# MougyTestspace/hclib

Measured on AMD Instinct MI355X. Metric: UTS nodes/sec (tasks/sec) at 1/2/4/8 MI355X vs host-CPU HClib; forasync HBM GB/s, higher is better.
Workload: dtype u32; 1 GPU; test/uts T3L (-t 0 -b 2000 -q 0.200014 -m 5 -r 7) searched whole on 1 GPU (no split); nodes=111345631, bit_exact=True, parallelism=shard1 (hash-partitioned frontier, RCCL all-reduce of counts)

## Files before the change

hclib_amd/__init__.py:

```python
from __future__ import annotations

import ctypes as C
import os
from typing import Optional, Tuple

PKG = os.path.dirname(os.path.abspath(__file__))
LIB_PATH = os.environ.get("HCLIB_AMD_LIB") or os.path.join(PKG, "lib", "libhclib_amd.so")

HCLIB_HIP_OK = 0
FORASYNC_MODE_FLAT = 0
FORASYNC_MODE_RECURSIVE = 1
BODY_TRIAD_F32 = 1
BODY_IOTA_CHECK = 2
BODY_VISIT_COUNT = 3


class HclibError(RuntimeError):
    pass


class LoopDomain(C.Structure):

    _fields_ = [("low", C.c_int), ("high", C.c_int), ("stride", C.c_int), ("tile", C.c_int)]

# ... 77 lines not shown


class StrassenResult(C.Structure):

    _fields_ = [("tasks", C.c_uint64), ("splits", C.c_uint64), ("base", C.c_uint64), ("tiles", C.c_uint64),
                ("pre_bands", C.c_uint64), ("combine_bands", C.c_uint64), ("finishes", C.c_uint64),
                ("check_ins", C.c_uint64), ("workspace_bytes", C.c_uint64),
                ("kernel_ms", C.c_double), ("gflops", C.c_double)]


class AtomicViewStruct(C.Structure):

    _fields_ = [("slots", C.c_void_p), ("nslots", C.c_uint32), ("stride", C.c_uint32),
                ("dtype", C.c_int), ("op", C.c_int)]


EXPORTS_HIP = [
    "hclib_hip_init", "hclib_hip_finalize", "hclib_hip_device_memory_live", "hclib_hip_last_error",
    "hclib_hip_num_cus",
    "hclib_hip_version", "hclib_hip_forasync", "hclib_hip_forasync_triad_f32",
    "hclib_hip_num_workers", "hclib_hip_uts_search", "hclib_hip_uts_num_children_host",
    "hclib_hip_uts_bucket_check", "hclib_hip_sha1_calibrate",
    "hclib_hip_fib", "hclib_hip_sw", "hclib_hip_last_sched_counters", "hclib_hip_last_narrow_counters",
    "hclib_hip_last_phase_counters",
    "hclib_hip_sw_band_begin", "hclib_hip_sw_band_rows", "hclib_hip_sw_band_end",
    "hclib_hip_atomic_create", "hclib_hip_atomic_destroy", "hclib_hip_atomic_view",
    "hclib_hip_atomic_gather", "hclib_hip_atomic_gather_async", "hclib_hip_atomic_reset",
    "hclib_hip_forasync_reduce", "hclib_hip_cholesky", "hclib_hip_sort_i64", "hclib_hip_sort_bounds",
    "hclib_hip_sparselu_genmat", "hclib_hip_sparselu_plan", "hclib_hip_sparselu", "hclib_hip_sparselu_bmod_rate",
    "hclib_hip_nqueens", "hclib_hip_nqueens_bounds",
    "hclib_hip_strassen", "hclib_hip_strassen_bounds", "hclib_hip_strassen_last_ticks",
    "hclib_atomic_create", "hclib_atomic_init", "hclib_atomic_update", "hclib_atomic_gather",
]

_lib = None


def lib():
    global _lib
    if _lib is None:
        try:
            import torch
        except ImportError:
            pass
        if not os.path.exists(LIB_PATH):
            raise HclibError(f"{LIB_PATH} is missing: run `python -m hclib_amd.build`")
        L = C.CDLL(LIB_PATH)
# ... 566 lines not shown
    _check(lib().hclib_hip_sha1_calibrate(chains, waves_per_cu, iters, C.byref(r), C.byref(ms)),
           "hclib_hip_sha1_calibrate")
    return r.value, ms.value


def last_phase_counters():
    out = (C.c_uint64 * 8)()
    lib().hclib_hip_last_phase_counters(out)
    return list(out)


def last_sched_counters():
    out = (C.c_uint64 * 16)()
    lib().hclib_hip_last_sched_counters(out)
    return list(out)


def last_narrow_counters():
    out = (C.c_uint64 * 4)()
    lib().hclib_hip_last_narrow_counters(out)
    return list(out)


TIMELINE_EVENTS = {1: "start", 2: "busy", 3: "idle", 4: "spill", 5: "term", 6: "end"}


def last_timeline():
    per = C.c_uint32()
    nw = lib().hclib_hip_last_timeline(None, 0, C.byref(per))
    if nw <= 0 or per.value == 0:
        return []
    import numpy as np
    buf = np.zeros(nw * per.value, dtype=np.uint64)
    lib().hclib_hip_last_timeline(buf.ctypes.data, buf.size, C.byref(per))
    buf = buf.reshape(nw, per.value)
    out = []
    for w in range(nw):
        row = buf[w][buf[w] != 0]
        out.append([(int(v >> 24), int((v >> 20) & 0xF), int(v & 0xFFFFF)) for v in row])
    return out
```

hclib_amd/csrc/hx_module.h:

```cpp
#pragma once

#include <hip/hip_runtime.h>
#include <stdint.h>

#include <string>
#include <vector>

#include "../../include/hclib_hip.h"
#include "../../include/hclib_hip/hx_sched.h"

namespace hx {

enum ArenaId {
    kArenaGlobals,
    kArenaWaveStats,
    kArenaWaveCtr,
    kArenaTimeline,
    kArenaDeques,
    kArenaSeed,
    kArenaDag,
    kArenaDagTrace,
    kArenaDyn,
    kArenaCholesky,
    kArenaSparselu,
    kArenaSort,
    kArenaStrassen,
    kArenaUtsTables,
    kArenaCount
};
struct Arena {
    void *mem = nullptr;
    size_t bytes = 0;
};

struct Module {
    bool inited = false;
    int device = -1;
    int num_cus = 0;
    std::string arch;
    hipStream_t stream = nullptr;
    hipEvent_t ev0 = nullptr, ev1 = nullptr;
    Arena arenas[kArenaCount];
    bool uts_tables_cached = false;
    SchedGlobals *globals = nullptr;
    unsigned long long last_counters[16] = {};
    unsigned long long last_narrow[4] = {};
    unsigned long long last_phase[8] = {};
    WaveStat *wave_stats = nullptr;
    uint32_t wave_stats_cap = 0;
    std::vector<WaveStat> last_waves;
    unsigned long long *wave_ctr = nullptr;
    uint32_t rec_workers = 0;
    GlobalView gview = {nullptr, nullptr, nullptr, 0, 0};
    unsigned long long *timeline = nullptr;
    uint32_t timeline_cap = 0;
    std::vector<unsigned long long> last_timeline;
};

Module &mod();
void set_error(const char *fmt, ...);
int ensure_device();
int hip_check(hipError_t e, const char *what);
int check_resident(const void *kern, int blocks, int threads, size_t lds, const char *what);
int upload_async(void *dst, const void *src, size_t bytes, hipStream_t stream);

int arena_reserve(ArenaId id, size_t bytes, const char *who, void **ptr);

class DevBuf {
  public:
// ... 31 lines not shown
```

hclib_amd/csrc/module.hip:

```cpp
#include <stdarg.h>
#include <stdio.h>
#include <stdlib.h>
#include <string.h>

#include "hx_module.h"

namespace hx {

static Module g_mod;
static thread_local char g_err[512] = "";

Module &mod() { return g_mod; }

void set_error(const char *fmt, ...) {
    va_list ap;
    va_start(ap, fmt);
    vsnprintf(g_err, sizeof(g_err), fmt, ap);
    va_end(ap);
}

static uint64_t g_live[2] = {0, 0};
static bool dev_acquire(void **p, size_t bytes) {
    if (hipMalloc(p, bytes) != hipSuccess) {
        (void)hipGetLastError();
// ... 211 lines not shown

int finish_sched(SchedGlobals *host_copy, const char *who) {
    Module &m = g_mod;
    HX_HIP(hipMemcpyAsync(host_copy, m.globals, sizeof(SchedGlobals), hipMemcpyDeviceToHost,
                          m.stream));
    const uint32_t nw_cap = m.wave_stats_cap;
    static std::vector<unsigned long long> rec;
    const uint32_t nrec = m.rec_workers;
    for (int i = 0; i < 8; ++i) m.last_phase[i] = 0;
    m.rec_workers = 0;
    if (nrec) {
        rec.resize((size_t)nrec * kWaveCtrWords);
        HX_HIP(hipMemcpyAsync(rec.data(), m.wave_ctr, rec.size() * 8, hipMemcpyDeviceToHost, m.stream));
    }
    HX_HIP(hipStreamSynchronize(m.stream));
    for (uint32_t w = 0; w < nrec; ++w) {
        const unsigned long long *r = &rec[(size_t)w * kWaveCtrWords];
        for (int i = 0; i < 16; ++i)
            if (i >= 8 || i < 4) host_copy->counters[i] += r[i];
        for (int i = 4; i < 8; ++i) host_copy->counters[i] += r[24 + i - 4];
        for (int i = 0; i < 4; ++i)
            if (r[16 + i] > host_copy->maxes[i]) host_copy->maxes[i] = r[16 + i];
        for (int i = 0; i < 3; ++i) host_copy->narrow[i] += r[20 + i];
        m.last_phase[0] += r[23];
        for (int i = 0; i < 4; ++i) m.last_phase[1 + i] += r[28 + i];
        m.last_phase[5] += r[24];
        m.last_phase[6] += r[27];
    }
    memcpy(m.last_counters, host_copy->counters, sizeof(m.last_counters));
    memcpy(m.last_narrow, host_copy->narrow, sizeof(m.last_narrow));
    uint64_t nw = host_copy->counters[kCtrWaves];
    if (nw > nw_cap) nw = nw_cap;
    m.last_waves.resize(nw);
    if (nw) HX_HIP(hipMemcpy(m.last_waves.data(), m.wave_stats, nw * sizeof(WaveStat), hipMemcpyDeviceToHost));
    if (host_copy->timeline) {
        m.last_timeline.resize((size_t)nw * m.timeline_cap);
        if (nw)
            HX_HIP(hipMemcpy(m.last_timeline.data(), m.timeline, (size_t)nw * m.timeline_cap * 8,
                             hipMemcpyDeviceToHost));
    } else {
        m.last_timeline.clear();
    }
    if (host_copy->err) {
        set_error("%s: device error %u (%s)", who, host_copy->err, err_name(host_copy->err));
        return HCLIB_HIP_EDEVICE;
    }
    return HCLIB_HIP_OK;
}

}

using namespace hx;

// ... 50 lines not shown
}

void hclib_hip_device_memory_live(uint64_t out[2]) {
    out[0] = g_live[0];
    out[1] = g_live[1];
}

int hclib_hip_num_cus(void) { return g_mod.inited ? g_mod.num_cus : 0; }

int hclib_hip_device(void) { return g_mod.inited ? g_mod.device : -1; }

void *hclib_hip_stream(void) { return g_mod.inited ? (void *)g_mod.stream : nullptr; }

void hclib_hip_last_sched_counters(uint64_t out[16]) {
    for (int i = 0; i < 16; ++i) out[i] = g_mod.last_counters[i];
}

extern "C" void hclib_hip_last_phase_counters(uint64_t out[8]) {
    for (int i = 0; i < 8; ++i) out[i] = g_mod.last_phase[i];
}

void hclib_hip_last_narrow_counters(uint64_t out[4]) {
    for (int i = 0; i < 4; ++i) out[i] = g_mod.last_narrow[i];
}

int hclib_hip_last_wave_stats(hclib_hip_wave_stats_t *out, int max) {
    static_assert(sizeof(hclib_hip_wave_stats_t) == sizeof(WaveStat), "layout");
    const int n = (int)g_mod.last_waves.size();
    for (int i = 0; out && i < n && i < max; ++i) memcpy(&out[i], &g_mod.last_waves[(size_t)i], sizeof(WaveStat));
    return n;
}

int hclib_hip_last_timeline(uint64_t *out, uint64_t max_words, uint32_t *events_per_worker) {
    Module &m = g_mod;
    if (events_per_worker) *events_per_worker = m.last_timeline.empty() ? 0u : m.timeline_cap;
    const uint64_t n = m.last_timeline.size();
    for (uint64_t i = 0; out && i < n && i < max_words; ++i) out[i] = m.last_timeline[i];
    return m.timeline_cap ? (int)(n / m.timeline_cap) : 0;
}

int hclib_hip_sched_begin(uint32_t entry_words, uint32_t chunk, int waves_per_cu,
                          hclib_hip_sched_launch_t *out) {
    if (!out || entry_words < 4 || entry_words > 64 || waves_per_cu < 1 || waves_per_cu > 8) {
        set_error("hclib_hip_sched_begin: invalid arguments");
        return HCLIB_HIP_EINVAL;
    }
// ... 183 lines not shown
```

hclib_amd/csrc/uts.hip:

```cpp
#include <math.h>
#include <string.h>

#include <type_traits>
#include <vector>

#include "hx_module.h"
#include "uts_sha1.h"

namespace hx {

#define HX_ROTL(x, n) (((x) << (n)) | ((x) >> (32 - (n))))
#define HX_RND(f, k, wi)                                \
    {                                                   \
        uint32_t t_ = HX_ROTL(a, 5) + (f) + e + (k) + (wi); \
        e = d;                                          \
        d = c;                                          \
        c = HX_ROTL(b, 30);                             \
        b = a;                                          \
        a = t_;                                         \
    }
#define HX_F1 (d ^ (b & (c ^ d)))
#define HX_F2 (b ^ c ^ d)
#define HX_F3 ((b & c) | (d & (b ^ c)))
#define HX_W(i) \
// ... 731 lines not shown
    }
    const bool seeded = seed_fits;
    if (seeded) spill_lo_default = uts_expected_nodes(*params) >= 3e7 ? 448 : 336;
    {
        const int ring_launch = bin ? 1024 : ring_used, lo = env_int("HCLIB_HIP_SPILL_LO", spill_lo_default);
        if (lo < 1 || lo > ring_launch) {
            set_error("hclib_hip_uts_search: HCLIB_HIP_SPILL_LO=%d does not fit the %d-item ring of this launch "
                      "(1..%d)", lo, ring_launch, ring_launch);
            return HCLIB_HIP_EINVAL;
        }
    }
    cfg.spill_lo = (uint32_t)env_int("HCLIB_HIP_SPILL_LO", spill_lo_default);
    cfg.spin_limit = (uint32_t)env_int("HCLIB_HIP_SPIN_LIMIT_MS", 20000);
    cfg.nwaves = (uint32_t)grid;
    cfg.stamps = (uint32_t)env_int("HCLIB_HIP_STAMPS", 0);
    const bool small_fixed = geo_fixed && uts_expected_nodes(*params) < 3e7;
    const bool large_fixed = geo_fixed && ring_used >= 512 && !small_fixed;
    cfg.hunger = (uint32_t)env_int("HCLIB_HIP_HUNGER", large_fixed ? 128 : bin ? 64 : 32);
    cfg.carry = (uint32_t)env_int("HCLIB_HIP_CARRY", 2);
    cfg.backoff = (uint32_t)env_int("HCLIB_HIP_BACKOFF", 16);
    cfg.defer = (uint32_t)env_int("HCLIB_HIP_DEFER", 1);
    cfg.dual = (uint32_t)env_int("HCLIB_HIP_UTS_DUAL", 1);
    cfg.spills = (uint32_t)env_int("HCLIB_HIP_SPILLS_PER_BATCH", 0);
    SeedCfg seed{0, 0, (uint32_t)UtsKind<kUtsBin, 0>::kWords, 0};
    if (seeded) {
        seed.target = (uint32_t)(grid * per_wave);
        seed.max_levels = (uint32_t)env_int("HCLIB_HIP_SEED_LEVELS", 20);
        seed.solo_cap = (uint32_t)env_int("HCLIB_HIP_SEED_SOLO", 128);
        if (nshards > 1) {
            double n_split = 1.0, n_next = 1.0;
            for (int d = 0; d <= split_depth && d < 64; ++d) {
                if (d < split_depth) n_split *= geo_bi(*params, d) > 0 ? geo_bi(*params, d) : 0.0;
                n_next *= geo_bi(*params, d) > 0 ? geo_bi(*params, d) : 0.0;
            }
            const double cap = 8.0 * seed.target + 65536.0;
            const bool fits = split_depth + 1 < kSeedMaxLevels && split_depth < (int)seed.max_levels &&
                              n_split <= 0.5 * cap && n_next / nshards <= (double)grid * (512 / 8);
            seed.min_levels = fits ? (uint32_t)split_depth : 0u;
        }
    } else if (bin_seed) {
        seed.target = 1;
        seed.max_levels = (uint32_t)split_depth;
        seed.min_levels = (uint32_t)split_depth;
    }
    HX_TRY(reset_sched(pool, 1, global, (uint32_t)grid, seed.target ? &seed : nullptr));
    HX_HIP(hipEventRecord(m.ev0, m.stream));
// ... 78 lines not shown
```

include/hclib_hip.h:

```cpp
#ifndef HCLIB_HIP_H_
#define HCLIB_HIP_H_

#include <stddef.h>
#include <stdint.h>

#ifdef __cplusplus
extern "C" {
#endif

#define HCLIB_HIP_OK 0
#define HCLIB_HIP_ENODEV (-1)
#define HCLIB_HIP_EINVAL (-2)
#define HCLIB_HIP_ENOMEM (-3)
#define HCLIB_HIP_EDEVICE (-4)
#define HCLIB_HIP_EHIP (-5)

int hclib_hip_init(int device);
void hclib_hip_finalize(void);
void hclib_hip_device_memory_live(uint64_t out[2]);
const char *hclib_hip_last_error(void);
int hclib_hip_num_cus(void);
int hclib_hip_device(void);
void *hclib_hip_stream(void);
const char *hclib_hip_version(void);
void hclib_hip_last_sched_counters(uint64_t out[16]);

typedef struct {
    uint64_t executed;
    uint64_t spawned;
    uint64_t batches;
    uint64_t chunks_pushed;
    uint64_t chunks_stolen;
    uint64_t items_stolen;
    uint64_t xcd;
    uint64_t reserved;
    uint64_t stolen_from[8];
} hclib_hip_wave_stats_t;
int hclib_hip_last_wave_stats(hclib_hip_wave_stats_t *out, int max);
void hclib_hip_last_narrow_counters(uint64_t out[4]);
void hclib_hip_last_phase_counters(uint64_t out[8]);
int hclib_hip_last_timeline(uint64_t *out, uint64_t max_words, uint32_t *events_per_worker);

#define HCLIB_HIP_ATOMIC_SCATTER_RET64 0
#define HCLIB_HIP_ATOMIC_HOT_WORD 1
#define HCLIB_HIP_ATOMIC_COALESCED32 2
int hclib_hip_atomic_calibrate(int mode, int iters, double *mops_per_s, double *kernel_ms);
int hclib_hip_sparselu_bmod_rate(int B, int wgs_per_cu, int reps, double *ms, double *gflops);
int hclib_hip_sha1_calibrate(int chains, int waves_per_cu, int iters, double *sha1_per_s, double *kernel_ms);

typedef struct {
    void *hdr;
    uint32_t *seq;
    uint32_t *cnt;
    uint32_t *data;
    uint32_t nq, cap, chunk;
    void *globals;
    void *stream;
    int grid;
    int num_cus;
} hclib_hip_sched_launch_t;

int hclib_hip_sched_begin(uint32_t entry_words, uint32_t chunk, int waves_per_cu,
// ... 272 lines not shown
```

include/hclib_hip/hx_sched.h:

```cpp
#pragma once

#include <type_traits>

#include "hx_common.h"

namespace hx {

constexpr int kWaveSize = 64;

struct alignas(256) QueueHdr {
    uint32_t head;
    uint32_t done;
    uint32_t pad0[30];
    uint32_t tail;
    uint32_t pad1[31];
};

struct WaveStat {
    unsigned long long executed, spawned, batches, chunks_pushed, chunks_stolen, items_stolen;
    unsigned long long xcd;
    unsigned long long reserved;
    unsigned long long stolen_from[8];
};
static_assert(sizeof(WaveStat) == 128, "WaveStat is 16 words");
// ... 29 lines not shown
    uint32_t pad1[63];
    uint32_t hints[8 * 64];
    uint32_t err;
    uint32_t pad2[63];
    unsigned long long counters[16];
    unsigned long long maxes[4];
    WaveStat *wave_stats;
    uint32_t wave_stats_cap;
    unsigned long long narrow[4];
    GlobalView gview;
    unsigned long long *timeline;
    uint32_t timeline_cap;
    unsigned long long *wave_ctr;
    uint32_t wave_ctr_cap;
    struct Seed {
        uint32_t *buf;
        uint32_t *ctl;
        uint32_t cap;
        uint32_t target;
        uint32_t max_levels;
        uint32_t min_levels;
        uint32_t solo_cap;
    } seed;
};
constexpr int kSeedMaxLevels = 24;
constexpr int kSeedGoLines = 64;
constexpr int kSeedCtlLines = 2 * kSeedMaxLevels + 2 + kSeedGoLines;
constexpr int kWaveCtrWords = 32;

#ifndef HX_TIMELINE
#define HX_TIMELINE 0
#endif
enum : uint32_t {
    kTlStart = 1,
    kTlBusy = 2,
    kTlIdle = 3,
    kTlSpill = 4,
    kTlTerm = 5,
    kTlEnd = 6,
    kTlProbe = 7,
    kTlSeed = 8,
};
struct Timeline {
    unsigned long long *p;
    uint32_t n, cap;
    __device__ __forceinline__ void init(SchedGlobals *g, uint32_t worker) {
#if HX_TIMELINE
        cap = g->timeline_cap;
        p = g->timeline ? g->timeline + (size_t)worker * cap : nullptr;
        n = 0;
#endif
// ... 30 lines not shown
struct PoolView {
    QueueHdr *hdr;
    uint32_t *seq;
    uint32_t *cnt;
    uint32_t *data;
    uint32_t nq;
    uint32_t cap;
    uint32_t chunk;
};

struct SchedConfig {
    uint32_t spill_hi;
    uint32_t spill_lo;
    uint32_t spin_limit;
    uint32_t nwaves;
    uint32_t stamps;
    uint32_t hunger;
    uint32_t backoff = 16;
    uint32_t carry = 2;
    uint32_t defer = 1;
    uint32_t dual = 1;
    uint32_t spills = 0;
    uint32_t hunger_init_full = 0;
};


constexpr uint32_t kResidualSplitMin = 2;

template <class K, class = void>
struct KindHasSeedProcess {
    static constexpr bool value = false;
};
template <class K>
struct KindHasSeedProcess<K, decltype((void)&K::seed_process)> {
    static constexpr bool value = true;
};
template <class K>
__device__ __forceinline__ int kind_seed_process(const typename K::Ctx &c, typename K::Acc &acc, const uint32_t *t,
                                                 uint32_t k, uint32_t *child, uint32_t *err, bool valid) {
    if constexpr (KindHasSeedProcess<K>::value) return K::seed_process(c, acc, t, k, child, err, valid);
    else return K::process(c, acc, t, k, child, err, valid);
}

template <class K, class = void>
struct KindPieces {
    static constexpr int value = 8;
// ... 12 lines not shown
struct KindHasDual<K, decltype((void)&K::process2)> {
    static constexpr bool value = K::kPure;
};
template <class K>
constexpr int group_max_of() { return KindPieces<K>::value + 2; }
template <class K, class = void>
struct KindFixedChildren {
    static constexpr bool value = false;
};
template <class K, class = void>
struct KindBulkCount {
    static constexpr bool value = false;
};
template <class K>
struct KindBulkCount<K, decltype((void)K::kBulkCount)> {
    static constexpr bool value = K::kBulkCount;
};
template <class K>
struct KindFixedChildren<K, decltype((void)K::kFixedChildren)> {
    static constexpr bool value = K::kFixedChildren;
};
constexpr uint32_t kMaxChildren = 1u << 24;

template <class Kind, int CAP>
struct WaveStack {
    static constexpr int TW = Kind::kTmplWords;
    static_assert(TW == 2 || TW == 6, "templates are 2 or 6 words");
    static_assert((CAP & (CAP - 1)) == 0, "CAP must be a power of two");
    uint2 d[CAP];
    uint4 t0[TW == 6 ? CAP : 1];
    uint2 t1[CAP];
    uint32_t mark[64];
    uint32_t stolen_from[8];
    unsigned long long cyc[6];
    static constexpr bool kCarryLds = CAP >= 1024;
    uint4 cscr[kCarryLds ? 128 : 1];
};

template <class WS>
__device__ __forceinline__ void lds_sum(WS &st, int i, unsigned long long v) {
    if (lane_id() == 0) __hip_atomic_fetch_add(&st.cyc[i], v, __ATOMIC_RELAXED, __HIP_MEMORY_SCOPE_WAVEFRONT);
}

template <class Kind, int CAP>
__device__ __forceinline__ void load_tmpl(const WaveStack<Kind, CAP> &st, uint32_t slot, uint32_t *t) {
    if constexpr (Kind::kTmplWords == 6) {
        const uint4 a = st.t0[slot];
        const uint2 b = st.t1[slot];
// ... 399 lines not shown
__device__ __forceinline__ uint32_t rcp16(uint32_t mu) {
    return mu <= 4 ? (mu <= 2 ? (mu == 1 ? 65536u : 32768u) : (mu == 3 ? 21846u : 16384u))
                   : (mu <= 6 ? (mu == 5 ? 13108u : 10923u) : (mu == 7 ? 9363u : 8192u));
}

template <int TW>
__device__ __forceinline__ void carry_permute(unsigned long long spawn, uint32_t mu, uint32_t nch,
                                              const uint32_t *child, uint32_t *ctmpl, uint32_t &ck,
                                              uint32_t rcp = 0) {
    const uint32_t lane = (uint32_t)lane_id();
    const uint32_t nsp = (uint32_t)__builtin_popcountll(spawn);
    const uint32_t rk = (uint32_t)__builtin_amdgcn_mbcnt_hi((uint32_t)(spawn >> 32),
                                                           __builtin_amdgcn_mbcnt_lo((uint32_t)spawn, 0u));
    const uint32_t dst = nch != 0 ? rk : nsp + (lane - rk);
    const int src_of_rank = __builtin_amdgcn_ds_permute((int)(dst * 4u), (int)lane);
    const uint32_t r = __umul24(lane, rcp ? rcp : rcp16(mu)) >> 16;
    const int src = __builtin_amdgcn_ds_bpermute((int)(r * 4u), src_of_rank);
#pragma unroll
    for (int i = 0; i < TW; ++i) ctmpl[i] = (uint32_t)__builtin_amdgcn_ds_bpermute(src * 4, (int)child[i]);
    ck = lane - __umul24(r, mu);
}

template <int TW>
__device__ __forceinline__ void carry_lds_slot(uint4 *scr, unsigned long long spawn, bool mine, const uint32_t *child,
                                               uint32_t *ctmpl, uint32_t r) {
    const uint32_t rk = (uint32_t)__builtin_amdgcn_mbcnt_hi((uint32_t)(spawn >> 32),
                                                           __builtin_amdgcn_mbcnt_lo((uint32_t)spawn, 0u));
    if (mine) {
        if constexpr (TW == 6) {
            scr[2 * rk] = make_uint4(child[0], child[1], child[2], child[3]);
            *(uint2 *)&scr[2 * rk + 1] = make_uint2(child[4], child[5]);
        } else {
            *(uint2 *)&scr[2 * rk] = make_uint2(child[0], child[1]);
        }
    }
    if constexpr (TW == 6) {
        const uint4 a = scr[2 * r];
        const uint2 b = *(const uint2 *)&scr[2 * r + 1];
        ctmpl[0] = a.x;
        ctmpl[1] = a.y;
        ctmpl[2] = a.z;
        ctmpl[3] = a.w;
        ctmpl[4] = b.x;
        ctmpl[5] = b.y;
    } else {
        const uint2 a = *(const uint2 *)&scr[2 * r];
        ctmpl[0] = a.x;
        ctmpl[1] = a.y;
    }
}

template <int TW>
__device__ __forceinline__ void carry_lds(uint4 *scr, unsigned long long spawn, uint32_t mu, const uint32_t *child,
                                          uint32_t *ctmpl, uint32_t &ck, uint32_t rcp = 0) {
    const uint32_t lane = (uint32_t)lane_id();
    const uint32_t r = __umul24(lane, rcp ? rcp : rcp16(mu)) >> 16;
    carry_lds_slot<TW>(scr, spawn, ((spawn >> lane) & 1ull) != 0, child, ctmpl, r);
    ck = lane - __umul24(r, mu);
}

template <class Kind, int CAP>
__device__ __forceinline__ void push_uniform(WaveStack<Kind, CAP> &st, uint32_t base, uint32_t excl,
                                             uint32_t tout, uint32_t mu, bool spawned,
                                             const uint32_t *child) {
    constexpr uint32_t M = CAP - 1;
    if (spawned) store_tmpl<Kind, CAP>(st, (base + excl) & M, child);
    const uint32_t rcp = rcp16(mu);
    for (uint32_t r0 = 0; r0 < tout; r0 += kWaveSize) {
        const uint32_t o = r0 + (uint32_t)lane_id();
        if (o < tout) {
            const uint32_t kk = o - ((o * rcp) >> 16) * mu;
            st.d[(base + o) & M] = make_uint2(kk, (kk + 1) | (kk << 24));
// ... 85 lines not shown
#endif
template <class A, class = void>
struct acc_has_mode : std::false_type {};
template <class A>
struct acc_has_mode<A, decltype((void)A::mode)> : std::true_type {};
template <class A>
__device__ __forceinline__ void acc_set_mode(A &a, uint32_t m) {
    if constexpr (acc_has_mode<A>::value) a.mode = m;
}
template <class A, class = void>
struct acc_has_totals : std::false_type {};
template <class A>
struct acc_has_totals<A, decltype((void)&A::totals)> : std::true_type {};

template <class A, class = void>
struct acc_has_wid : std::false_type {};
template <class A>
struct acc_has_wid<A, decltype((void)A::wid)> : std::true_type {};
template <class A>
__device__ __forceinline__ void acc_set_wid(A &a, uint32_t w) {
    if constexpr (acc_has_wid<A>::value) a.wid = w;
}

template <class Kind, int CAP>
__device__ __forceinline__ NarrowState<Kind::kTmplWords> narrow_loop_fixed(
    const typename Kind::Ctx &ctx_ref, typename Kind::Acc &acc_ref, uint32_t *err, WaveStack<Kind, CAP> &st,
    NarrowState<Kind::kTmplWords> ns, uint32_t mu, uint32_t r_fix, uint32_t ck_fix) {
    constexpr int TW = Kind::kTmplWords;
    const typename Kind::Ctx ctx = ctx_ref;
    typename Kind::Acc acc = acc_ref;
    acc_set_mode(acc, 1u);
    const uint32_t lane = (uint32_t)lane_id();
    constexpr bool kBulk = KindBulkCount<Kind>::value;
    uint32_t carry = lane0(ns.carry), batches = 0, s_exec = 0, s_nsp = 0, t2;
    const uint32_t k = ck_fix;
    uint32_t ch2[TW];
    bool sp;
    unsigned long long sp2;
    do {
        const bool h = lane < carry;
        if constexpr (kBulk) sp = Kind::process_bulk(ctx, acc, ns.ctmpl, k, ch2, err, h);
        else sp = Kind::process(ctx, acc, ns.ctmpl, k, ch2, err, h) > 0;
        ++batches;
        s_exec += carry;
        sp2 = __builtin_amdgcn_ballot_w64(sp);
        const uint32_t nsp = (uint32_t)__builtin_popcountll(sp2);
        s_nsp += nsp;
        t2 = mu * nsp;
        carry_lds_slot<TW>(st.cscr, sp2, sp, ch2, ns.ctmpl, r_fix);
        carry = t2;
    } while (t2 - 1u < (uint32_t)kWaveSize);
    ns.ck = ck_fix;
    if (t2 != 0) {
        const uint32_t rk2 = (uint32_t)__builtin_amdgcn_mbcnt_hi(
            (uint32_t)(sp2 >> 32), __builtin_amdgcn_mbcnt_lo((uint32_t)sp2, 0u));
        push_uniform<Kind, CAP>(st, ns.top, mu * rk2, t2, mu, sp, ch2);
        ns.top += t2;
        carry = 0;
    }
    if constexpr (kBulk) Kind::count_bulk(acc, s_exec, s_exec - s_nsp);
    if (lane == 0) {
        ns.n_exec += s_exec;
        ns.n_spawn += mu * s_nsp;
    }
    ns.carry = carry;
    ns.batches = batches;
    acc_set_mode(acc, 0u);
    acc_ref = acc;
    return ns;
}

template <class Kind, int CAP>
__device__ __forceinline__ NarrowState<Kind::kTmplWords> narrow_loop(
    const typename Kind::Ctx &ctx_ref, typename Kind::Acc &acc_ref, uint32_t *err, WaveStack<Kind, CAP> &st,
    NarrowState<Kind::kTmplWords> ns) {
    constexpr int TW = Kind::kTmplWords;
    constexpr int kPieces = pieces_of<Kind>();
    const typename Kind::Ctx ctx = ctx_ref;
    typename Kind::Acc acc = acc_ref;
    acc_set_mode(acc, 1u);
    const uint32_t lane = (uint32_t)lane_id();
    uint32_t carry = lane0(ns.carry), batches = 0;
    uint32_t mu_fix = 0, rcp_fix = 0;
    if constexpr (KindFixedChildren<Kind>::value) {
        mu_fix = lane0(Kind::fixed_children(ctx));
        if (mu_fix > (uint32_t)kPieces) mu_fix = 0;
        rcp_fix = mu_fix ? rcp16(mu_fix) : 0u;
    }
    const bool hoist = mu_fix != 0;
    const uint32_t r_fix = hoist ? __umul24(lane, rcp_fix) >> 16 : 0u;
    const uint32_t ck_fix = hoist ? lane - __umul24(r_fix, mu_fix) : 0u;
    if constexpr (KindFixedChildren<Kind>::value && Kind::kPure && Kind::kBoundedChildren &&
                  WaveStack<Kind, CAP>::kCarryLds) {
        if (hoist) return narrow_loop_fixed<Kind, CAP>(ctx_ref, acc_ref, err, st, ns, mu_fix, r_fix, ck_fix);
    }
    while (true) {
        const bool h = lane < carry;
        uint32_t ch2[TW];
        int c2 = 0;
        if constexpr (Kind::kPure) {
            c2 = Kind::process(ctx, acc, ns.ctmpl, ns.ck, ch2, err, h);
        } else {
            if (h) c2 = Kind::process(ctx, acc, ns.ctmpl, ns.ck, ch2, err, true);
        }
        ++batches;
        uint32_t u2 = c2 > 0 ? (uint32_t)c2 : 0u;
        if (!Kind::kBoundedChildren && u2 >= kMaxChildren) {
            dev_error(err, kErrBadTask);
            u2 = 0;
        }
        ns.n_exec += h ? 1u : 0u;
        ns.n_spawn += h ? u2 : 0u;
        const uint32_t n2 = u2 > (uint32_t)kPieces ? (uint32_t)kPieces : u2;
        const unsigned long long sp2 = __ballot(n2 != 0);
        if (!sp2) {
            carry = 0;
            break;
// ... 33 lines not shown
                                    ns.ck + 1, ns.tag);
            ns.tag += 16;
            ns.top += t2;
        }
        carry = 0;
        break;
    }
    ns.carry = carry;
    ns.batches = batches;
    acc_set_mode(acc, 0u);
    acc_ref = acc;
    return ns;
}

template <class Kind>
struct Inbox {
    uint32_t state;
    uint32_t n;
    uint32_t idle;
    uint32_t pad;
    uint32_t w[64 * Kind::kWords];
};

template <class Kind, int CAP>
__device__ bool inbox_put(const typename Kind::Ctx &ctx, Inbox<Kind> &ib, WaveStack<Kind, CAP> &st, uint32_t bot,
                          uint32_t n, SchedGlobals *g) {
    constexpr int W = Kind::kWords;
    const int lane = lane_id();
    const bool valid = (uint32_t)lane < n;
    const uint32_t p = bot + (valid ? (uint32_t)lane : 0u);
    const uint2 dd = st.d[p & (CAP - 1)];
    uint32_t ok = 0;
    if (lane == 0) ok = lds_cas(&ib.state, 0u, 2u) ? 1u : 0u;
    uint32_t w[W];
    load_tmpl<Kind, CAP>(st, (p - (dd.y >> 24)) & (CAP - 1), w);
    if (!lane0(ok)) return false;
    {
        w[W - 2] = dd.x;
        w[W - 1] = dd.y & (kMaxChildren - 1);
        kind_export<Kind>(ctx, w, valid, &g->err);
        kind_trace_item<Kind>(ctx, w, valid, 2u, true);
        if (valid) {
#pragma unroll
            for (int i = 0; i < W; ++i) ib.w[(uint32_t)lane * W + i] = w[i];
        }
    }
    asm volatile("" ::: "memory");
    if (lane == 0) {
        add_agent(&g->outstanding, 1u);
        lds_store(&ib.n, n);
        lds_store(&ib.idle, 0u);
        lds_store(&ib.state, 1u);
    }
    return true;
}

template <class Kind, int CAP>
__device__ uint32_t inbox_take(const typename Kind::Ctx &ctx, Inbox<Kind> &ib, WaveStack<Kind, CAP> &st) {
    constexpr int W = Kind::kWords;
    const int lane = lane_id();
    if (lane0(lds_load(&ib.state)) != 1u) return 0;
    const uint32_t n = lane0(lds_load(&ib.n));
    if ((uint32_t)lane < n) {
        uint32_t w[W];
#pragma unroll
        for (int i = 0; i < W; ++i) w[i] = ib.w[(uint32_t)lane * W + i];
        store_tmpl<Kind, CAP>(st, (uint32_t)lane, w);
        st.d[lane] = make_uint2(w[W - 2], w[W - 1]);
        kind_trace_item<Kind>(ctx, w, true, 3u, true);
    }
    if (lane == 0) lds_store(&ib.state, 0u);
    return n;
}

template <bool GLOBAL>
__device__ __forceinline__ void wave_goes_idle(SchedGlobals *g, const GlobalView &gv, const PoolView &pool) {
    if (lane_id() != 0) return;
// ... 241 lines not shown
    const uint32_t qpx = pool.nq / 8;
    const uint32_t xcc = xcc_id() & 7u;
    const uint32_t home = xcc * qpx + (gid / 8) % qpx;
    uint32_t rng = 0x9e3779b9u ^ (gid * 0x85ebca6bu + 1u);

    typename Kind::Acc acc;
    acc_set_wid(acc, gid);
    Timeline tl;
    tl.init(g, gid);
    tl.log(kTlStart, 0);
    ProbeStats pstat;
    uint32_t bot = 0, top = 0;
    bool active = false;
    uint32_t spins = 0;
    unsigned long long idle_since = 0;
    uint32_t nbatch = 0, npush = 0, nsteal = 0;
    unsigned long long cyc_form = 0, cyc_proc = 0, cyc_push = 0;
    unsigned long long ph_sum[6] = {0, 0, 0, 0, 0, 0}, ph_n = 0, ph_a = 0, ph_b = 0, ph_c = 0, ph_d = 0, ph_m = 0,
                       ph_p = 0;
    bool ph_single = false;
    uint32_t tag = 1;
    for (int i = lane; i < kWaveSize; i += kWaveSize) st.mark[i] = 0;
    if (lane < 8) st.stolen_from[lane] = 0;
    uint32_t n_exec = 0, n_spawn = 0;
    uint32_t items_stolen = 0;
    uint32_t n_narrow = 0, n_narrow_in = 0;
    uint32_t carry = 0, ck = 0;
    uint32_t ctmpl[TW];
    PendingChunk pend;
    pend.live = false;
    uint32_t occ = 0;
#pragma unroll
    for (int i = 0; i < TW; ++i) ctmpl[i] = 0;

    bool seeded = false;
    if constexpr (Kind::kPure && Kind::kTmplWords == 6 && Kind::kWords == 8 && CAP >= 128) {
        if (g->seed.buf) {
            seeded = true;
            top = seed_levels<Kind, CAP>(ctx, acc, g, st, gid, cfg.nwaves, cfg.spin_limit, n_exec, n_spawn, nbatch, tl);
            st.mark[lane] = 0;
            active = true;
            tl.log(kTlBusy, top);
            if (top == 0) {
                active = false;
                wave_goes_idle<GLOBAL>(g, gv, pool);
            }
// ... 365 lines not shown
            excl = (uint32_t)(P - nout);
        }
        {
            const uint32_t hungry0 = cfg.nwaves > outst ? cfg.nwaves - outst : 0;
            if (cfg.carry && uniform && tout > 0 && tout <= (uint32_t)kWaveSize &&
                !(hungry0 > 0 && (top - bot) + tout >= cfg.spill_lo)) {
                if constexpr (WaveStack<Kind, CAP>::kCarryLds) carry_lds<TW>(st.cscr, spawn, mu, child, ctmpl, ck);
                else carry_permute<TW>(spawn, mu, nch, child, ctmpl, ck);
                carry = tout;
                if (HX_STAMPS && cfg.stamps) cyc_push += __builtin_amdgcn_s_memtime() - ts0;
                if (HX_STAMPS && cfg.stamps) t_batch = __builtin_amdgcn_s_memtime();
                if (cfg.carry > 1 && top == bot && cfg.spill_lo > (uint32_t)kWaveSize && !(HX_STAMPS && cfg.stamps)) {
                    const unsigned long long tn0 = __builtin_amdgcn_s_memtime();
                    NarrowState<TW> ns;
#pragma unroll
                    for (int i = 0; i < TW; ++i) ns.ctmpl[i] = ctmpl[i];
                    ns.ck = ck;
                    ns.carry = carry;
                    ns.top = top;
                    ns.tag = tag;
                    ns.n_exec = n_exec;
                    ns.n_spawn = n_spawn;
                    ns.batches = 0;
                    ns = narrow_loop<Kind, CAP>(ctx, acc, &g->err, st, ns);
#pragma unroll
                    for (int i = 0; i < TW; ++i) ctmpl[i] = ns.ctmpl[i];
                    ck = ns.ck;
                    carry = lane0(ns.carry);
                    top = lane0(ns.top);
                    tag = lane0(ns.tag);
                    n_exec = ns.n_exec;
                    n_spawn = ns.n_spawn;
                    nbatch += lane0(ns.batches);
                    n_narrow += lane0(ns.batches);
                    lds_sum(st, 3, __builtin_amdgcn_s_memtime() - tn0);
                    ++n_narrow_in;
                }
                continue;
            }
        }
        if (HX_PHASES) ph_m = __builtin_amdgcn_s_memtime();
        if (!make_room(tout)) break;
        if (uniform) {
            push_uniform<Kind, CAP>(st, top, excl, tout, mu, nch != 0, child);
        } else {
            push_outputs<Kind, CAP>(st, top, excl, tout, nres, ucnt, nch, tmpl, child, k, kend, tag);
            tag += 16;
// ... 59 lines not shown
            const unsigned long long ph_e = __builtin_amdgcn_s_memtime();
            ph_sum[0] += ph_b - ph_a;
            ph_sum[1] += ph_c - ph_b;
            ph_sum[2] += ph_d - ph_c;
            ph_sum[3] += ph_e - ph_d;
            ph_sum[4] += ph_m - ph_d;
            ph_sum[5] += ph_p - ph_m;
            ++ph_n;
        }
    }
    publish_pending<Kind, CAP>(pool, g, pend);
    if constexpr (WPG > 1) {
        if (lane == 0) {
            lds_store(&ib[wave].idle, 0u);
            (void)lds_cas(&ib[wave].state, 0u, 3u);
        }
    }
    const unsigned long long t_end = __builtin_amdgcn_s_memtime();
    const unsigned long long rt_end = __builtin_amdgcn_s_memrealtime();
    lds_sum(st, busy_phase ? 0 : 1, t_end - t_mark);
    __builtin_amdgcn_s_waitcnt(0xC07F);
    const unsigned long long cyc_busy = st.cyc[0], cyc_idle = st.cyc[1], cyc_spill = st.cyc[2],
                             cyc_narrow = st.cyc[3], t_begin = st.cyc[4], rt_begin = st.cyc[5];
    if (active) {
        wave_goes_idle<GLOBAL>(g, gv, pool);
    }
    const bool rec = g->wave_ctr && gid < g->wave_ctr_cap;
    unsigned long long kc[8] = {0, 0, 0, 0, 0, 0, 0, 0}, km[4] = {0, 0, 0, 0};
    if constexpr (acc_has_totals<typename Kind::Acc>::value) {
        acc.totals(kc, km);
        if (!rec && lane == 0) {
            for (int i = 0; i < 8; ++i)
                if (kc[i]) add_agent(&g->counters[i], kc[i]);
            for (int i = 0; i < 4; ++i)
                if (km[i]) __hip_atomic_fetch_max(&g->maxes[i], km[i], __ATOMIC_RELAXED, HX_AGENT);
        }
    } else {
        acc.flush(g);
    }
    {
        const unsigned long long ex = wave_sum((unsigned long long)n_exec),
                                 sp = wave_sum((unsigned long long)n_spawn);
        if (g->wave_stats && gid < g->wave_stats_cap && lane < 16) {
            unsigned long long v = 0;
            switch (lane) {
            case 0: v = ex; break;
            case 1: v = sp; break;
            case 2: v = nbatch; break;
            case 3: v = npush; break;
            case 4: v = nsteal; break;
            case 5: v = items_stolen; break;
            case 6: v = xcc; break;
            case 7: v = 0; break;
            default: v = st.stolen_from[lane - 8]; break;
            }
            ((unsigned long long *)&g->wave_stats[gid])[lane] = v;
        }
    }
    const unsigned long long c_push = (HX_STAMPS && cfg.stamps) ? cyc_push - cyc_proc : 0,
                             c_form = (HX_STAMPS && cfg.stamps) ? cyc_form : 0,
                             c_proc = (HX_STAMPS && cfg.stamps) ? cyc_proc : 0;
    if (rec) {
        unsigned long long v = 0;
#pragma unroll
        for (int i = 0; i < 8; ++i)
            if (lane == i) v = kc[i];
#pragma unroll
        for (int i = 0; i < 4; ++i)
            if (lane == 16 + i) v = km[i];
        switch (lane) {
        case 8 + kCtrProcCycles - 8: v = c_proc; break;
        case 8 + kCtrBusyCycles - 8: v = cyc_busy; break;
        case 8 + kCtrIdleCycles - 8: v = cyc_idle; break;
        case 8 + kCtrSpillCycles - 8: v = cyc_spill; break;
        case 8 + kCtrWaves - 8: v = 1; break;
        case 8 + kCtrBatches - 8: v = nbatch; break;
        case 8 + kCtrPushed - 8: v = npush; break;
        case 8 + kCtrStolen - 8: v = nsteal; break;
        case 20: v = n_narrow_in ? (unsigned long long)n_narrow : 0; break;
        case 21: v = n_narrow_in ? cyc_narrow : 0; break;
        case 22: v = n_narrow_in; break;
        case 23: v = ph_n; break;
        case 28: v = ph_sum[0]; break;
        case 29: v = ph_sum[1]; break;
        case 30: v = ph_sum[2]; break;
        case 31: v = ph_sum[3]; break;
        case 24 + kCtrPushCycles - 4: v = HX_PHASES ? ph_sum[4] : c_push; break;
        case 24 + kCtrClockTicks - 4: v = t_end - t_begin; break;
        case 24 + kCtrRealTicks - 4: v = rt_end - rt_begin; break;
        case 24 + kCtrFormCycles - 4: v = HX_PHASES ? ph_sum[5] : c_form; break;
        default: break;
        }
        if (lane < kWaveCtrWords) g->wave_ctr[(size_t)gid * kWaveCtrWords + lane] = v;
    } else {
        if (lane == 0 && n_narrow_in) {
            add_agent(&g->narrow[0], (unsigned long long)n_narrow);
            add_agent(&g->narrow[1], cyc_narrow);
            add_agent(&g->narrow[2], (unsigned long long)n_narrow_in);
        }
        if (lane == 0) {
            add_agent(&g->counters[kCtrBusyCycles], cyc_busy);
            if (HX_STAMPS && cfg.stamps) {
                add_agent(&g->counters[kCtrFormCycles], c_form);
                add_agent(&g->counters[kCtrProcCycles], c_proc);
                add_agent(&g->counters[kCtrPushCycles], c_push);
            }
            add_agent(&g->counters[kCtrIdleCycles], cyc_idle);
            add_agent(&g->counters[kCtrSpillCycles], cyc_spill);
            add_agent(&g->counters[kCtrWaves], 1ull);
            add_agent(&g->counters[kCtrBatches], (unsigned long long)nbatch);
            add_agent(&g->counters[kCtrPushed], (unsigned long long)npush);
            add_agent(&g->counters[kCtrStolen], (unsigned long long)nsteal);
            add_agent(&g->counters[kCtrClockTicks], t_end - t_begin);
            add_agent(&g->counters[kCtrRealTicks], rt_end - rt_begin);
        }
    }
    tl.log(kTlEnd, 0);
// ... 11 lines not shown
```

Measured before the change: 4.123 billion nodes/s.

## Shed narrow-loop spawns into idle sibling inboxes on narrow exit

When the fixed-children narrow loop exits with spawned children, the wave now keeps only part of them (half, a quarter, or what fits one carry pass, chosen by HCLIB_HIP_NARROW_SHED) and hands the rest straight to idle sibling waves' LDS inboxes in the same workgroup. If all the remaining children go to inboxes, the wave keeps running the narrow loop on the kept ones instead of pushing to its ring. The aim is to cut ring push traffic and idle time in sibling waves by redistributing work inside the workgroup. It adds LDS state reads, CAS claims and outstanding-counter atomics at every narrow exit, plus new shed counters that widen the per-wave counter record to 40 words.

```diff
diff --git a/hclib_amd/__init__.py b/hclib_amd/__init__.py
--- a/hclib_amd/__init__.py
+++ b/hclib_amd/__init__.py
@@ -123,7 +123,7 @@
     "hclib_hip_num_workers", "hclib_hip_uts_search", "hclib_hip_uts_num_children_host",
     "hclib_hip_uts_bucket_check", "hclib_hip_sha1_calibrate",
     "hclib_hip_fib", "hclib_hip_sw", "hclib_hip_last_sched_counters", "hclib_hip_last_narrow_counters",
-    "hclib_hip_last_phase_counters",
+    "hclib_hip_last_phase_counters", "hclib_hip_last_shed_counters",
     "hclib_hip_sw_band_begin", "hclib_hip_sw_band_rows", "hclib_hip_sw_band_end",
     "hclib_hip_atomic_create", "hclib_hip_atomic_destroy", "hclib_hip_atomic_view",
     "hclib_hip_atomic_gather", "hclib_hip_atomic_gather_async", "hclib_hip_atomic_reset",
@@ -736,6 +736,12 @@
     return list(out)
 
 
+def last_shed_counters():
+    out = (C.c_uint64 * 8)()
+    lib().hclib_hip_last_shed_counters(out)
+    return dict(zip(("exits", "placed", "blocks", "items", "fallbacks"), out))
+
+
 TIMELINE_EVENTS = {1: "start", 2: "busy", 3: "idle", 4: "spill", 5: "term", 6: "end"}
 
 
diff --git a/hclib_amd/csrc/hx_module.h b/hclib_amd/csrc/hx_module.h
--- a/hclib_amd/csrc/hx_module.h
+++ b/hclib_amd/csrc/hx_module.h
@@ -45,6 +45,7 @@
     SchedGlobals *globals = nullptr;
     unsigned long long last_counters[16] = {};
     unsigned long long last_narrow[4] = {};
+    unsigned long long last_shed[8] = {};
     unsigned long long last_phase[8] = {};
     WaveStat *wave_stats = nullptr;
     uint32_t wave_stats_cap = 0;
diff --git a/hclib_amd/csrc/module.hip b/hclib_amd/csrc/module.hip
--- a/hclib_amd/csrc/module.hip
+++ b/hclib_amd/csrc/module.hip
@@ -257,6 +257,7 @@
         for (int i = 0; i < 4; ++i)
             if (r[16 + i] > host_copy->maxes[i]) host_copy->maxes[i] = r[16 + i];
         for (int i = 0; i < 3; ++i) host_copy->narrow[i] += r[20 + i];
+        for (int i = 0; i < kShedCounts; ++i) host_copy->shed[i] += r[32 + i];
         m.last_phase[0] += r[23];
         for (int i = 0; i < 4; ++i) m.last_phase[1 + i] += r[28 + i];
         m.last_phase[5] += r[24];
@@ -264,6 +265,7 @@
     }
     memcpy(m.last_counters, host_copy->counters, sizeof(m.last_counters));
     memcpy(m.last_narrow, host_copy->narrow, sizeof(m.last_narrow));
+    memcpy(m.last_shed, host_copy->shed, sizeof(m.last_shed));
     uint64_t nw = host_copy->counters[kCtrWaves];
     if (nw > nw_cap) nw = nw_cap;
     m.last_waves.resize(nw);
@@ -360,6 +362,10 @@
 
 void hclib_hip_last_narrow_counters(uint64_t out[4]) {
     for (int i = 0; i < 4; ++i) out[i] = g_mod.last_narrow[i];
+}
+
+void hclib_hip_last_shed_counters(uint64_t out[8]) {
+    for (int i = 0; i < 8; ++i) out[i] = g_mod.last_shed[i];
 }
 
 int hclib_hip_last_wave_stats(hclib_hip_wave_stats_t *out, int max) {
diff --git a/hclib_amd/csrc/uts.hip b/hclib_amd/csrc/uts.hip
--- a/hclib_amd/csrc/uts.hip
+++ b/hclib_amd/csrc/uts.hip
@@ -777,6 +777,15 @@
     cfg.defer = (uint32_t)env_int("HCLIB_HIP_DEFER", 1);
     cfg.dual = (uint32_t)env_int("HCLIB_HIP_UTS_DUAL", 1);
     cfg.spills = (uint32_t)env_int("HCLIB_HIP_SPILLS_PER_BATCH", 0);
+    {
+        const int rule = env_int("HCLIB_HIP_NARROW_SHED", 1), sibs = env_int("HCLIB_HIP_NARROW_SHED_SIBS", 3);
+        if (rule < 0 || rule > 3 || sibs < 0 || sibs > 3) {
+            set_error("hclib_hip_uts_search: HCLIB_HIP_NARROW_SHED=%d / HCLIB_HIP_NARROW_SHED_SIBS=%d: the keep rule is "
+                      "0 (off), 1, 2 or 3, the sibling inboxes per exit 0..3", rule, sibs);
+            return HCLIB_HIP_EINVAL;
+        }
+        cfg.narrow_shed = (uint32_t)rule | (uint32_t)sibs << 8;
+    }
     SeedCfg seed{0, 0, (uint32_t)UtsKind<kUtsBin, 0>::kWords, 0};
     if (seeded) {
         seed.target = (uint32_t)(grid * per_wave);
diff --git a/include/hclib_hip.h b/include/hclib_hip.h
--- a/include/hclib_hip.h
+++ b/include/hclib_hip.h
@@ -38,6 +38,7 @@
 } hclib_hip_wave_stats_t;
 int hclib_hip_last_wave_stats(hclib_hip_wave_stats_t *out, int max);
 void hclib_hip_last_narrow_counters(uint64_t out[4]);
+void hclib_hip_last_shed_counters(uint64_t out[8]);
 void hclib_hip_last_phase_counters(uint64_t out[8]);
 int hclib_hip_last_timeline(uint64_t *out, uint64_t max_words, uint32_t *events_per_worker);
 
diff --git a/include/hclib_hip/hx_sched.h b/include/hclib_hip/hx_sched.h
--- a/include/hclib_hip/hx_sched.h
+++ b/include/hclib_hip/hx_sched.h
@@ -75,11 +75,20 @@
         uint32_t min_levels;
         uint32_t solo_cap;
     } seed;
+    unsigned long long shed[8];
 };
 constexpr int kSeedMaxLevels = 24;
 constexpr int kSeedGoLines = 64;
 constexpr int kSeedCtlLines = 2 * kSeedMaxLevels + 2 + kSeedGoLines;
-constexpr int kWaveCtrWords = 32;
+constexpr int kWaveCtrWords = 40;
+enum : int {
+    kShedExits = 0,
+    kShedPlaced = 1,
+    kShedBlocks = 2,
+    kShedItems = 3,
+    kShedFallbacks = 4,
+    kShedCounts = 5,
+};
 
 #ifndef HX_TIMELINE
 #define HX_TIMELINE 0
@@ -156,6 +165,7 @@
     uint32_t dual = 1;
     uint32_t spills = 0;
     uint32_t hunger_init_full = 0;
+    uint32_t narrow_shed = 0;
 };
 
 
@@ -214,8 +224,19 @@
 };
 constexpr uint32_t kMaxChildren = 1u << 24;
 
+template <bool ON>
+struct ShedSlots {};
+template <>
+struct ShedSlots<true> {
+    unsigned long long shed_g;
+    uint32_t shed_ib;
+    uint32_t shed_wave;
+    uint32_t shed_cfg;
+    uint32_t shed_cnt[kShedCounts];
+};
+
 template <class Kind, int CAP>
-struct WaveStack {
+struct WaveStack : ShedSlots<(CAP >= 1024)> {
     static constexpr int TW = Kind::kTmplWords;
     static_assert(TW == 2 || TW == 6, "templates are 2 or 6 words");
     static_assert((CAP & (CAP - 1)) == 0, "CAP must be a power of two");
@@ -661,18 +682,7 @@
 }
 
 template <int TW>
-__device__ __forceinline__ void carry_lds_slot(uint4 *scr, unsigned long long spawn, bool mine, const uint32_t *child,
-                                               uint32_t *ctmpl, uint32_t r) {
-    const uint32_t rk = (uint32_t)__builtin_amdgcn_mbcnt_hi((uint32_t)(spawn >> 32),
-                                                           __builtin_amdgcn_mbcnt_lo((uint32_t)spawn, 0u));
-    if (mine) {
-        if constexpr (TW == 6) {
-            scr[2 * rk] = make_uint4(child[0], child[1], child[2], child[3]);
-            *(uint2 *)&scr[2 * rk + 1] = make_uint2(child[4], child[5]);
-        } else {
-            *(uint2 *)&scr[2 * rk] = make_uint2(child[0], child[1]);
-        }
-    }
+__device__ __forceinline__ void carry_lds_read(const uint4 *scr, uint32_t r, uint32_t *ctmpl) {
     if constexpr (TW == 6) {
         const uint4 a = scr[2 * r];
         const uint2 b = *(const uint2 *)&scr[2 * r + 1];
@@ -687,6 +697,21 @@
         ctmpl[0] = a.x;
         ctmpl[1] = a.y;
     }
+}
+template <int TW>
+__device__ __forceinline__ void carry_lds_slot(uint4 *scr, unsigned long long spawn, bool mine, const uint32_t *child,
+                                               uint32_t *ctmpl, uint32_t r) {
+    const uint32_t rk = (uint32_t)__builtin_amdgcn_mbcnt_hi((uint32_t)(spawn >> 32),
+                                                           __builtin_amdgcn_mbcnt_lo((uint32_t)spawn, 0u));
+    if (mine) {
+        if constexpr (TW == 6) {
+            scr[2 * rk] = make_uint4(child[0], child[1], child[2], child[3]);
+            *(uint2 *)&scr[2 * rk + 1] = make_uint2(child[4], child[5]);
+        } else {
+            *(uint2 *)&scr[2 * rk] = make_uint2(child[0], child[1]);
+        }
+    }
+    carry_lds_read<TW>(scr, r, ctmpl);
 }
 
 template <int TW>
@@ -818,7 +843,11 @@
     if constexpr (acc_has_wid<A>::value) a.wid = w;
 }
 
-template <class Kind, int CAP>
+template <class Kind, int CAP, int WPG>
+__device__ __forceinline__ uint32_t narrow_shed(const typename Kind::Ctx &ctx, WaveStack<Kind, CAP> &st, uint32_t mu,
+                                                uint32_t nsp, uint32_t r_fix, uint32_t ck_fix, uint32_t &to_ring);
+
+template <class Kind, int CAP, int WPG = 1>
 __device__ __forceinline__ NarrowState<Kind::kTmplWords> narrow_loop_fixed(
     const typename Kind::Ctx &ctx_ref, typename Kind::Acc &acc_ref, uint32_t *err, WaveStack<Kind, CAP> &st,
     NarrowState<Kind::kTmplWords> ns, uint32_t mu, uint32_t r_fix, uint32_t ck_fix) {
@@ -833,6 +862,7 @@
     uint32_t ch2[TW];
     bool sp;
     unsigned long long sp2;
+    while (true) {
     do {
         const bool h = lane < carry;
         if constexpr (kBulk) sp = Kind::process_bulk(ctx, acc, ns.ctmpl, k, ch2, err, h);
@@ -846,14 +876,19 @@
         carry_lds_slot<TW>(st.cscr, sp2, sp, ch2, ns.ctmpl, r_fix);
         carry = t2;
     } while (t2 - 1u < (uint32_t)kWaveSize);
+    if (t2 == 0) break;
+    const uint32_t nsp = (uint32_t)__builtin_popcountll(sp2);
+    uint32_t kept = 0, to_ring = 0;
+    if constexpr (WPG > 1) kept = narrow_shed<Kind, CAP, WPG>(ctx, st, mu, nsp, r_fix, ck_fix, to_ring);
+    carry = mu * kept;
+    if (kept != 0 && to_ring == nsp) continue;
+    const uint32_t rk2 = (uint32_t)__builtin_amdgcn_mbcnt_hi(
+        (uint32_t)(sp2 >> 32), __builtin_amdgcn_mbcnt_lo((uint32_t)sp2, 0u));
+    push_uniform<Kind, CAP>(st, ns.top, mu * (rk2 - to_ring), mu * (nsp - to_ring), mu, sp && rk2 >= to_ring, ch2);
+    ns.top += mu * (nsp - to_ring);
+    break;
+    }
     ns.ck = ck_fix;
-    if (t2 != 0) {
-        const uint32_t rk2 = (uint32_t)__builtin_amdgcn_mbcnt_hi(
-            (uint32_t)(sp2 >> 32), __builtin_amdgcn_mbcnt_lo((uint32_t)sp2, 0u));
-        push_uniform<Kind, CAP>(st, ns.top, mu * rk2, t2, mu, sp, ch2);
-        ns.top += t2;
-        carry = 0;
-    }
     if constexpr (kBulk) Kind::count_bulk(acc, s_exec, s_exec - s_nsp);
     if (lane == 0) {
         ns.n_exec += s_exec;
@@ -866,7 +901,7 @@
     return ns;
 }
 
-template <class Kind, int CAP>
+template <class Kind, int CAP, int WPG = 1>
 __device__ __forceinline__ NarrowState<Kind::kTmplWords> narrow_loop(
     const typename Kind::Ctx &ctx_ref, typename Kind::Acc &acc_ref, uint32_t *err, WaveStack<Kind, CAP> &st,
     NarrowState<Kind::kTmplWords> ns) {
@@ -888,7 +923,7 @@
     const uint32_t ck_fix = hoist ? lane - __umul24(r_fix, mu_fix) : 0u;
     if constexpr (KindFixedChildren<Kind>::value && Kind::kPure && Kind::kBoundedChildren &&
                   WaveStack<Kind, CAP>::kCarryLds) {
-        if (hoist) return narrow_loop_fixed<Kind, CAP>(ctx_ref, acc_ref, err, st, ns, mu_fix, r_fix, ck_fix);
+        if (hoist) return narrow_loop_fixed<Kind, CAP, WPG>(ctx_ref, acc_ref, err, st, ns, mu_fix, r_fix, ck_fix);
     }
     while (true) {
         const bool h = lane < carry;
@@ -968,6 +1003,33 @@
     uint32_t w[64 * Kind::kWords];
 };
 
+template <class Kind>
+__device__ __forceinline__ uint32_t inbox_claim(Inbox<Kind> &ib) {
+    uint32_t ok = 0;
+    if (lane_id() == 0) ok = lds_cas(&ib.state, 0u, 2u) ? 1u : 0u;
+    return ok;
+}
+
+template <class Kind>
+__device__ __forceinline__ void inbox_fill(const typename Kind::Ctx &ctx, Inbox<Kind> &ib, uint32_t *w, bool valid,
+                                           uint32_t n, SchedGlobals *g) {
+    constexpr int W = Kind::kWords;
+    kind_export<Kind>(ctx, w, valid, &g->err);
+    kind_trace_item<Kind>(ctx, w, valid, 2u, true);
+    if (valid) {
+        hx_lds_u32 *dst = (hx_lds_u32 *)&ib.w[(uint32_t)lane_id() * W];
+#pragma unroll
+        for (int i = 0; i < W; ++i) dst[i] = w[i];
+    }
+    asm volatile("" ::: "memory");
+    if (lane_id() == 0) {
+        add_agent(&g->outstanding, 1u);
+        lds_store(&ib.n, n);
+        lds_store(&ib.idle, 0u);
+        lds_store(&ib.state, 1u);
+    }
+}
+
 template <class Kind, int CAP>
 __device__ bool inbox_put(const typename Kind::Ctx &ctx, Inbox<Kind> &ib, WaveStack<Kind, CAP> &st, uint32_t bot,
                           uint32_t n, SchedGlobals *g) {
@@ -976,29 +1038,67 @@
     const bool valid = (uint32_t)lane < n;
     const uint32_t p = bot + (valid ? (uint32_t)lane : 0u);
     const uint2 dd = st.d[p & (CAP - 1)];
-    uint32_t ok = 0;
-    if (lane == 0) ok = lds_cas(&ib.state, 0u, 2u) ? 1u : 0u;
+    const uint32_t ok = inbox_claim<Kind>(ib);
     uint32_t w[W];
     load_tmpl<Kind, CAP>(st, (p - (dd.y >> 24)) & (CAP - 1), w);
     if (!lane0(ok)) return false;
-    {
-        w[W - 2] = dd.x;
-        w[W - 1] = dd.y & (kMaxChildren - 1);
-        kind_export<Kind>(ctx, w, valid, &g->err);
-        kind_trace_item<Kind>(ctx, w, valid, 2u, true);
-        if (valid) {
+    w[W - 2] = dd.x;
+    w[W - 1] = dd.y & (kMaxChildren - 1);
+    inbox_fill<Kind>(ctx, ib, w, valid, n, g);
+    return true;
+}
+
+template <class Kind, int CAP, int WPG>
+__device__ __forceinline__ uint32_t narrow_shed(const typename Kind::Ctx &ctx, WaveStack<Kind, CAP> &st, uint32_t mu,
+                                                uint32_t nsp, uint32_t r_fix, uint32_t ck_fix, uint32_t &to_ring) {
+    constexpr int TW = Kind::kTmplWords, W = Kind::kWords;
+    const uint32_t lane = (uint32_t)lane_id();
+    to_ring = 0;
+    const uint32_t cfg = lane0(lds_load(&st.shed_cfg));
+    const uint32_t rule = cfg & 0xffu, max_blocks = (cfg >> 8) & 0xffu;
+    if (rule == 0) return 0;
+    const uint32_t fit = (64u * rcp16(mu)) >> 16;
+    uint32_t keep = rule == 2 ? fit : (rule == 3 ? nsp / 4 : nsp / 2);
+    keep = keep > fit ? fit : (keep == 0 ? 1u : keep);
+    const uint32_t wave = lane0(lds_load(&st.shed_wave));
+    typedef __attribute__((address_space(3))) Inbox<Kind> lds_inbox;
+    Inbox<Kind> *ib = (Inbox<Kind> *)(lds_inbox *)(uintptr_t)lane0(lds_load(&st.shed_ib));
+    const unsigned long long gp = st.shed_g;
+    SchedGlobals *g = (SchedGlobals *)(((unsigned long long)lane0((uint32_t)(gp >> 32)) << 32) | lane0((uint32_t)gp));
+    uint32_t sid[WPG], sst[WPG];
 #pragma unroll
-            for (int i = 0; i < W; ++i) ib.w[(uint32_t)lane * W + i] = w[i];
-        }
-    }
-    asm volatile("" ::: "memory");
+    for (uint32_t a = 1; a < (uint32_t)WPG; ++a) {
+        sid[a] = lds_load(&ib[(wave + a) % (uint32_t)WPG].idle);
+        sst[a] = lds_load(&ib[(wave + a) % (uint32_t)WPG].state);
+    }
+    const uint32_t nshed = nsp - keep;
+    uint32_t placed = 0, blocks = 0;
+#pragma unroll
+    for (uint32_t a = 1; a < (uint32_t)WPG; ++a) {
+        if (placed < nshed && blocks < max_blocks && lane0(sid[a]) == 1u && lane0(sst[a]) == 0u) {
+            Inbox<Kind> &to = ib[(wave + a) % (uint32_t)WPG];
+            const uint32_t bs = nshed - placed < fit ? nshed - placed : fit, n = bs * mu;
+            const bool valid = lane < n;
+            const uint32_t ok = inbox_claim<Kind>(to);
+            uint32_t w[W];
+            carry_lds_read<TW>(st.cscr, keep + placed + (valid ? r_fix : 0u), w);
+            if (lane0(ok)) {
+                w[W - 2] = ck_fix;
+                w[W - 1] = ck_fix + 1u;
+                inbox_fill<Kind>(ctx, to, w, valid, n, g);
+                placed += bs;
+                ++blocks;
+            }
+        }
+    }
+    to_ring = keep + placed;
     if (lane == 0) {
-        add_agent(&g->outstanding, 1u);
-        lds_store(&ib.n, n);
-        lds_store(&ib.idle, 0u);
-        lds_store(&ib.state, 1u);
-    }
-    return true;
+        st.shed_cnt[kShedExits] += 1u;
+        st.shed_cnt[placed == nshed ? kShedPlaced : kShedFallbacks] += 1u;
+        st.shed_cnt[kShedBlocks] += blocks;
+        st.shed_cnt[kShedItems] += placed * mu;
+    }
+    return keep;
 }
 
 template <class Kind, int CAP>
@@ -1286,6 +1386,16 @@
     uint32_t tag = 1;
     for (int i = lane; i < kWaveSize; i += kWaveSize) st.mark[i] = 0;
     if (lane < 8) st.stolen_from[lane] = 0;
+    constexpr bool kShed = WPG > 1 && WaveStack<Kind, CAP>::kCarryLds;
+    if constexpr (kShed) {
+        if (lane == 0) {
+            st.shed_g = (unsigned long long)(uintptr_t)g;
+            st.shed_ib = (uint32_t)(uintptr_t)(__attribute__((address_space(3))) Inbox<Kind> *)ib;
+            st.shed_wave = wave;
+            st.shed_cfg = cfg.narrow_shed;
+        }
+        if (lane < kShedCounts) st.shed_cnt[lane] = 0;
+    }
     uint32_t n_exec = 0, n_spawn = 0;
     uint32_t items_stolen = 0;
     uint32_t n_narrow = 0, n_narrow_in = 0;
@@ -1697,7 +1807,7 @@
                     ns.n_exec = n_exec;
                     ns.n_spawn = n_spawn;
                     ns.batches = 0;
-                    ns = narrow_loop<Kind, CAP>(ctx, acc, &g->err, st, ns);
+                    ns = narrow_loop<Kind, CAP, WPG>(ctx, acc, &g->err, st, ns);
 #pragma unroll
                     for (int i = 0; i < TW; ++i) ctmpl[i] = ns.ctmpl[i];
                     ck = ns.ck;
@@ -1803,6 +1913,10 @@
     __builtin_amdgcn_s_waitcnt(0xC07F);
     const unsigned long long cyc_busy = st.cyc[0], cyc_idle = st.cyc[1], cyc_spill = st.cyc[2],
                              cyc_narrow = st.cyc[3], t_begin = st.cyc[4], rt_begin = st.cyc[5];
+    unsigned long long shed_v = 0;
+    if constexpr (kShed) {
+        if (lane >= 32 && lane < 32 + kShedCounts) shed_v = st.shed_cnt[lane - 32];
+    }
     if (active) {
         wave_goes_idle<GLOBAL>(g, gv, pool);
     }
@@ -1842,7 +1956,7 @@
                              c_form = (HX_STAMPS && cfg.stamps) ? cyc_form : 0,
                              c_proc = (HX_STAMPS && cfg.stamps) ? cyc_proc : 0;
     if (rec) {
-        unsigned long long v = 0;
+        unsigned long long v = shed_v;
 #pragma unroll
         for (int i = 0; i < 8; ++i)
             if (lane == i) v = kc[i];
@@ -1874,6 +1988,7 @@
         }
         if (lane < kWaveCtrWords) g->wave_ctr[(size_t)gid * kWaveCtrWords + lane] = v;
     } else {
+        if (shed_v) add_agent(&g->shed[lane - 32], shed_v);
         if (lane == 0 && n_narrow_in) {
             add_agent(&g->narrow[0], (unsigned long long)n_narrow);
             add_agent(&g->narrow[1], cyc_narrow);
```

Measured after the change: 4.368 billion nodes/s, median of 6. 5.9% higher.
